# hagabbar/GenNet

Hardware: AMD Instinct MI355X
Metric: waveforms/sec (CNN+GAN step, 2048-sample BBH) (higher is better)
Workload: dtype f32

## Files before the change

### gennet_amd/csrc/conv_epilogue.h

```cpp
#pragma once
#include "common.h"
#ifndef GN_STORE_AUX
#define GN_STORE_AUX 0
#endif

namespace gn {

typedef float f32x16 __attribute__((ext_vector_type(16)));

struct EpiSrd {
  __amdgpu_buffer_rsrc_t y, m, g;
  float ginv;
};
template <int MODE>
__device__ __forceinline__ EpiSrd epi_srd(const ConvArgs& a, int b) {
  EpiSrd s;
  const uintptr_t yp = (uintptr_t)(a.y + (size_t)b * a.Ly * a.Cout);
  const unsigned ylo = __builtin_amdgcn_readfirstlane((unsigned)yp), yhi = __builtin_amdgcn_readfirstlane((unsigned)(yp >> 32));
  const int ybytes = __builtin_amdgcn_readfirstlane(a.Ly * a.Cout * 4);
  s.y = __builtin_amdgcn_make_buffer_rsrc((void*)(((uintptr_t)yhi << 32) | ylo), 0, ybytes, 0x00020000);
  s.m = s.y; s.g = s.y;
  if (MODE == 1 || MODE == 3) {
    const uintptr_t mp = (uintptr_t)((MODE == 1 ? a.mask : a.gmask) + (size_t)b * a.Ly * a.Cout);
    const unsigned mlo = __builtin_amdgcn_readfirstlane((unsigned)mp), mhi = __builtin_amdgcn_readfirstlane((unsigned)(mp >> 32));
// ... 10 lines not shown
template <int ACT, int MODE, int GACT>
__device__ __forceinline__ void epi_store(const ConvArgs& a, const EpiSrd& s, float v, int voff, int soff) {
  if (ACT == GN_ACT_RELU) v = fmaxf(v, 0.f);
  else if (ACT == GN_ACT_LEAKY) v = v > 0.f ? v : a.act_param * v;
  else if (ACT == GN_ACT_TANH) v = gn_tanhf(v);
  else if (ACT != GN_ACT_LINEAR) v = act_apply(v, a.act, a.act_param);
  if (MODE == 1) {
    const unsigned k = __builtin_amdgcn_raw_buffer_load_b8(s.m, voff, soff, 0);
    v = k ? v * a.keep_scale : 0.f;
  }
  if (MODE >= 2) {
    const float gv = __builtin_bit_cast(float, __builtin_amdgcn_raw_buffer_load_b32(s.g, voff * 4, soff * 4, 0));
    if (MODE == 3) {
      const unsigned k = __builtin_amdgcn_raw_buffer_load_b8(s.m, voff, soff, 0);
      const float y0 = gv * s.ginv;
      const float dg = GACT == GN_ACT_LEAKY ? (y0 > 0.f ? 1.f : a.gparam) : act_grad_from_y(y0, a.gact, a.gparam);
      v = k ? v * a.gscale * dg : 0.f;
    } else {
      v *= GACT == GN_ACT_RELU ? (gv > 0.f ? 1.f : 0.f) : act_grad_from_y(gv, a.gact, a.gparam);
    }
  }
  __builtin_amdgcn_raw_buffer_store_b32(__builtin_bit_cast(unsigned, v), s.y, voff * 4, soff * 4, GN_STORE_AUX);
}

template <int ACT, int MODE, int GACT, int WN, int WMT = 2>
__device__ __forceinline__ void pipe_epilogue(const ConvArgs& a, const f32x16 (&acc)[WMT][WN], int b, int m_base, int n_base, int i32, int h, int out_off) {
  const EpiSrd srd = epi_srd<MODE>(a, b);
  const int rowstride = a.t.out_stride * a.Cout;
#pragma unroll
  for (int nt = 0; nt < WN; ++nt) {
    const int n = n_base + nt * 32 + i32;
    const float bias = a.bias ? a.bias[n] : 0.f;
    const int voff = rowstride * (4 * h) + out_off * a.Cout + n;
#pragma unroll
    for (int mt = 0; mt < WMT; ++mt) {
#pragma unroll
      for (int r = 0; r < 16; ++r) {
        const int soff = rowstride * (m_base + mt * 32 + (r & 3) + 8 * (r >> 2));
        epi_store<ACT, MODE, GACT>(a, srd, acc[mt][nt][r] + bias, voff, soff);
      }
    }
  }
}

typedef float f32x4e __attribute__((ext_vector_type(4)));
template <int ACT, int MODE, int GACT, int NT4>
// ... 14 lines not shown
                                                         int mode) {
#define GN_EPI(A_, M_, G_) tile16_epilogue<A_, M_, G_, NT4>(a, acc, b, m_base, n_base, n16, kq, out_off)
  if (mode == 0) {
    switch (a.act) {
      case GN_ACT_LINEAR: GN_EPI(GN_ACT_LINEAR, 0, -1); break;
      case GN_ACT_RELU: GN_EPI(GN_ACT_RELU, 0, -1); break;
      case GN_ACT_LEAKY: GN_EPI(GN_ACT_LEAKY, 0, -1); break;
      case GN_ACT_TANH: GN_EPI(GN_ACT_TANH, 0, -1); break;
      default: GN_EPI(-1, 0, -1); break;
    }
  } else if (mode == 1) {
    if (a.act == GN_ACT_LEAKY) GN_EPI(GN_ACT_LEAKY, 1, -1);
    else GN_EPI(-1, 1, -1);
  } else if (mode == 2) {
    if (a.act == GN_ACT_LINEAR && a.gact == GN_ACT_RELU) GN_EPI(GN_ACT_LINEAR, 2, GN_ACT_RELU);
    else GN_EPI(-1, 2, -1);
  } else {
    if (a.act == GN_ACT_LINEAR && a.gact == GN_ACT_LEAKY) GN_EPI(GN_ACT_LINEAR, 3, GN_ACT_LEAKY);
    else GN_EPI(-1, 3, -1);
  }
#undef GN_EPI
}

template <int WN, int WMT = 2>
__device__ __forceinline__ void pipe_epilogue_dispatch(const ConvArgs& a, const f32x16 (&acc)[WMT][WN], int b, int m_base, int n_base, int i32, int h, int out_off,
                                                       int mode) {
#define GN_EPI(A_, M_, G_) pipe_epilogue<A_, M_, G_, WN, WMT>(a, acc, b, m_base, n_base, i32, h, out_off)
  if (mode == 0) {
    switch (a.act) {
      case GN_ACT_LINEAR: GN_EPI(GN_ACT_LINEAR, 0, -1); break;
      case GN_ACT_RELU: GN_EPI(GN_ACT_RELU, 0, -1); break;
      case GN_ACT_LEAKY: GN_EPI(GN_ACT_LEAKY, 0, -1); break;
      case GN_ACT_TANH: GN_EPI(GN_ACT_TANH, 0, -1); break;
      default: GN_EPI(-1, 0, -1); break;
    }
  } else if (mode == 1) {
    if (a.act == GN_ACT_LEAKY) GN_EPI(GN_ACT_LEAKY, 1, -1);
    else GN_EPI(-1, 1, -1);
  } else if (mode == 2) {
    if (a.act == GN_ACT_LINEAR && a.gact == GN_ACT_RELU) GN_EPI(GN_ACT_LINEAR, 2, GN_ACT_RELU);
    else GN_EPI(-1, 2, -1);
  } else {
    if (a.act == GN_ACT_LINEAR && a.gact == GN_ACT_LEAKY) GN_EPI(GN_ACT_LINEAR, 3, GN_ACT_LEAKY);
    else GN_EPI(-1, 3, -1);
  }
#undef GN_EPI
// ... 32 lines not shown
```

### gennet_amd/csrc/conv_wino.hip

```cpp
#include <stdlib.h>
#include <algorithm>
#include <type_traits>
#include "common.h"
#include "conv_epilogue.h"
#include "wino_common.h"

namespace gn {

struct WinoTaps {
  int wq[5];
};

__global__ void wino_u_kernel(const float* __restrict__ w, float* __restrict__ U, int Cin, int Cout, WinoTaps t) {
  const size_t i = (size_t)blockIdx.x * blockDim.x + threadIdx.x;
  const size_t cc = (size_t)Cin * Cout;
  if (i >= cc) return;
  const int ci = (int)(i / Cout), co = (int)(i % Cout);
  double g[5];
#pragma unroll
  for (int q = 0; q < 5; ++q) g[q] = (double)w[(size_t)t.wq[q] * cc + i];
  float u[6];
  u[0] = (float)g[0];
  u[1] = (float)((g[0] + g[1] + g[2] + g[3] + g[4]) * (1.0 / 3.0));
  u[2] = (float)((g[0] - g[1] + g[2] - g[3] + g[4]) * (1.0 / 3.0));
  u[3] = (float)((16.0 * g[0] + 8.0 * g[1] + 4.0 * g[2] + 2.0 * g[3] + g[4]) * (1.0 / 15.0));
  u[4] = (float)((g[0] - 2.0 * g[1] + 4.0 * g[2] - 8.0 * g[3] + 16.0 * g[4]) * (1.0 / 30.0));
  u[5] = (float)g[4];
  const int chunk = ci >> 3, c = ci & 7, kq = c >> 1, s = c & 1;
  const int tile = co >> 6, nn = co & 63, ct = nn >> 4, n16 = nn & 15, cth = ct >> 1, ctl = ct & 1;
  const size_t base = ((size_t)chunk * (Cout >> 6) + tile) * 3072 + ((cth * 4 + kq) * 16 + n16) * 4 + ctl * 2 + s;
#pragma unroll
  for (int p = 0; p < 6; ++p) U[base + p * 512] = u[p];
}

template <int O, int OP1>
__device__ __forceinline__ void wino_slot_rba(f32x4& c, float a, float b, f32x4& nb0, f32x4& nb1, unsigned addr_b, f32x2 (&d)[6], unsigned addr_a) {
  asm volatile(
      "ds_read_b128 %1, %11 offset:%13\n\t"
      "ds_read_b128 %2, %11 offset:%14\n\t"
      "ds_read_b64 %3, %12\n\t"
      "ds_read_b64 %4, %12 offset:%15\n\t"
      "ds_read_b64 %5, %12 offset:32\n\t"
      "ds_read_b64 %6, %12 offset:%16\n\t"
      "ds_read_b64 %7, %12 offset:64\n\t"
      "ds_read_b64 %8, %12 offset:%17\n\t"
      "s_waitcnt lgkmcnt(8)\n\t"
      "v_mfma_f32_16x16x4_f32 %0, %9, %10, %0"
      : "+v"(c), "=&v"(nb0), "=&v"(nb1), "=&v"(d[0]), "=&v"(d[1]), "=&v"(d[2]), "=&v"(d[3]), "=&v"(d[4]), "=&v"(d[5])
      : "v"(a), "v"(b), "v"(addr_b), "v"(addr_a), "i"(O), "i"(O + 1024), "i"(OP1), "i"(OP1 + 32), "i"(OP1 + 64)
      : "memory");
}
template <int O>
__device__ __forceinline__ void wino_slot_rbw(f32x4& c, float a, float b, f32x4& nb0, f32x4& nb1, unsigned addr_b, f32x2 (&d)[6]) {
  asm volatile(
      "ds_read_b128 %1, %11 offset:%12\n\t"
      "ds_read_b128 %2, %11 offset:%13\n\t"
      "s_waitcnt lgkmcnt(2)\n\t"
      "v_mfma_f32_16x16x4_f32 %0, %9, %10, %0"
      : "+v"(c), "=&v"(nb0), "=&v"(nb1), "+v"(d[0]), "+v"(d[1]), "+v"(d[2]), "+v"(d[3]), "+v"(d[4]), "+v"(d[5])
      : "v"(a), "v"(b), "v"(addr_b), "i"(O), "i"(O + 1024)
      : "memory");
}

template <int RPER, int ABL = 0>
struct WinoChunk {
  template <int NPIECES, int I = 0, class D>
  static __device__ __forceinline__ void run(f32x4 (&acc)[6][4], const f32x2 (&v)[6], f32x2 (&vn)[6], f32x2 (&d)[6], WinoT& t, f32x4 (&B)[2][2], unsigned addr_b,
                                             unsigned addr_b_next, unsigned addr_a, unsigned long long k15, unsigned long long km15, D& dma) {
    if constexpr (I < 48) {
      constexpr int P = I / 8, S = (I / 4) % 2, CT = I % 4;
      f32x4(&bc)[2] = B[P & 1];
      f32x4(&bn)[2] = B[(P + 1) & 1];
      const float bv = bc[CT >> 1][2 * (CT & 1) + S];
      const float av = v[P][S];
      if constexpr ((ABL & 8) != 0) wino_slot(acc[P][CT], av, bv);
      else if constexpr (I == 0) wino_slot_rba<2048, RPER * 32>(acc[0][0], av, bv, bn[0], bn[1], addr_b, d, addr_a);
      else if constexpr (I == 8) wino_slot_rbw<2 * 2048>(acc[1][0], av, bv, bn[0], bn[1], addr_b, d);
      else if constexpr (I == 40) wino_slot_rb<0, 2>(acc[5][0], av, bv, bn[0], bn[1], addr_b_next);
      else if constexpr (I % 8 == 0) wino_slot_rb<(P + 1) * 2048, 2>(acc[P][0], av, bv, bn[0], bn[1], addr_b);
      else wino_slot(acc[P][CT], av, bv);
      if constexpr ((I & 1) && (I >> 1) < NPIECES) dma(std::integral_constant<int, (I >> 1)>{});
      if constexpr (!(ABL & 2)) {
        if constexpr (I == 12) wino_run<0, 5>(d, vn, t, k15, km15);
        if constexpr (I == 24) wino_run<5, 10>(d, vn, t, k15, km15);
        if constexpr (I == 36) wino_run<10, kWinoPieces>(d, vn, t, k15, km15);
      }
      run<NPIECES, I + 1>(acc, v, vn, d, t, B, addr_b, addr_b_next, addr_a, k15, km15, dma);
    }
  }
};

template <int WAVES_M, int ABL = 0>
__global__ __launch_bounds__(64 * WAVES_M, (WAVES_M > 4 ? 1 : 2)) void conv_wino_kernel(ConvArgs a, const float* __restrict__ U, int off0, int m_tiles, int n_tiles,
                                                                                        int patch) {
#if defined(__HIP_DEVICE_COMPILE__)
  constexpr int KC = 8, NP = 6;
  constexpr int TT = WAVES_M * 16;
  constexpr int TN = 64;
  constexpr int NT = 64 * WAVES_M;
  constexpr int RPER = TT + 2;
  constexpr int SLAB = 2 * RPER * KC;
  constexpr int UT = NP * KC * TN;
  constexpr int BUF = SLAB + UT;
  constexpr int STAGE_BYTES = BUF * 4;
  extern __shared__ __attribute__((aligned(16))) float smem[];
  typedef __attribute__((address_space(3))) void* lptr_t;

  const int tid = threadIdx.x, lane = tid & 63, wave = tid >> 6;
  const int n16 = lane & 15, kq = lane >> 4;
  const BlockTile bt = xcd_block_tile(patch, m_tiles, n_tiles);
  const int n_tile = bt.n_tile, m_tile = bt.m_tile, b = bt.b;
  const int t0 = m_tile * TT, n0 = n_tile * TN;

  f32x4 acc[NP][4];
#pragma unroll
  for (int p = 0; p < NP; ++p)
#pragma unroll
    for (int ct = 0; ct < 4; ++ct)
#pragma unroll
      for (int r = 0; r < 4; ++r) acc[p][ct][r] = 0.f;

  const int t_base = 2 * t0 + off0;
  const uintptr_t xbp = (uintptr_t)(a.x + (size_t)b * a.Lin * a.Cin);
  const unsigned xb_lo = __builtin_amdgcn_readfirstlane((unsigned)xbp), xb_hi = __builtin_amdgcn_readfirstlane((unsigned)(xbp >> 32));
  const int xbytes = __builtin_amdgcn_readfirstlane(a.Lin * a.Cin * 4);
  const __amdgpu_buffer_rsrc_t xsrd = __builtin_amdgcn_make_buffer_rsrc((void*)(((uintptr_t)xb_hi << 32) | xb_lo), 0, xbytes, 0x00020000);

// ... 43 lines not shown
  };

  const unsigned lds0 = (unsigned)(uintptr_t)smem;
  const unsigned base_a = lds0 + (wave * 16 + n16) * 32 + kq * 8;
  const unsigned base_b = lds0 + SLAB * 4 + (kq * 16 + n16) * 16;
  const unsigned long long k15 = 0x3fc000003fc00000ull, km15 = 0xbfc00000bfc00000ull;

  const int n_chunks = a.Cin / KC;
  c_next = 0; st_next = 0; dma_all();
  c_next = min(1, n_chunks - 1); st_next = 1; dma_all();
  __syncthreads();

  f32x2 V0[6], V1[6], d[6];
  f32x4 Bq[2][2];
  WinoT tt;
  {
    const char* sb = reinterpret_cast<const char*>(smem);
#pragma unroll
    for (int j = 0; j < 6; ++j) d[j] = *reinterpret_cast<const f32x2*>(sb + (base_a - lds0) + (j & 1) * RPER * 32 + (j >> 1) * 32);
    wino_run<0, kWinoPieces>(d, V0, tt, k15, km15);
    Bq[0][0] = *reinterpret_cast<const f32x4*>(sb + (base_b - lds0));
    Bq[0][1] = *reinterpret_cast<const f32x4*>(sb + (base_b - lds0) + 1024);
  }
  int st = 0;
  in_loop = true;
  for (int ch = 0; ch < n_chunks; ch += 2) {
#pragma unroll
    for (int half = 0; half < 2; ++half) {
      if (half == 1 && ch + 1 >= n_chunks) break;
      const int st1 = st == 2 ? 0 : st + 1, st2 = st1 == 2 ? 0 : st1 + 1;
      c_next = min(ch + half + 2, n_chunks - 1);
      st_next = st2;
      const unsigned addr_a = base_a + st1 * STAGE_BYTES;
      const unsigned addr_b = base_b + st * STAGE_BYTES, addr_b_next = base_b + st1 * STAGE_BYTES;
      if (half == 0) WinoChunk<RPER, ABL>::template run<NPIECES>(acc, V0, V1, d, tt, Bq, addr_b, addr_b_next, addr_a, k15, km15, dma_piece);
      else WinoChunk<RPER, ABL>::template run<NPIECES>(acc, V1, V0, d, tt, Bq, addr_b, addr_b_next, addr_a, k15, km15, dma_piece);
      if constexpr (!(ABL & 4)) __syncthreads();
      st = st1;
    }
  }
  asm volatile("s_nop 15\n\ts_nop 7" : "+v"(acc[5][0]), "+v"(acc[5][1]), "+v"(acc[5][2]), "+v"(acc[5][3]));

  f32x4 out[2][4];
#pragma unroll
  for (int ct = 0; ct < 4; ++ct)
#pragma unroll
    for (int r = 0; r < 4; ++r) {
      out[0][ct][r] = (((acc[0][ct][r] + acc[1][ct][r]) + acc[2][ct][r]) + acc[3][ct][r]) + acc[4][ct][r];
      out[1][ct][r] = __builtin_fmaf(-2.f, acc[4][ct][r], __builtin_fmaf(0.5f, acc[3][ct][r], acc[1][ct][r] - acc[2][ct][r])) + acc[5][ct][r];
    }
  const int m_base = t0 + __builtin_amdgcn_readfirstlane(wave) * 16;
  const int mode = a.gy ? (a.gmask ? 3 : 2) : (a.mask ? 1 : 0);
  ConvArgs a2 = a;
  a2.t.out_stride = 2;
  tile16_epilogue_dispatch<4>(a2, out[0], b, m_base, n0, n16, kq, a.t.out_off, mode);
  tile16_epilogue_dispatch<4>(a2, out[1], b, m_base, n0, n16, kq, a.t.out_off + 1, mode);

  if (a.stat_part) {
    double* red = reinterpret_cast<double*>(smem);
#pragma unroll
    for (int ct = 0; ct < 4; ++ct) {
      const float bias = a.bias ? a.bias[n0 + ct * 16 + n16] : 0.f;
      double s1 = 0.0, s2 = 0.0;
#pragma unroll
      for (int ph = 0; ph < 2; ++ph)
#pragma unroll
        for (int r = 0; r < 4; ++r) {
          const int row = 2 * (m_base + 4 * kq + r) + ph;
          if (row < a.M) {
            const double v = (double)(out[ph][ct][r] + bias);
            s1 += v; s2 += v * v;
          }
        }
      s1 += __shfl_xor(s1, 16, 64); s2 += __shfl_xor(s2, 16, 64);
      s1 += __shfl_xor(s1, 32, 64); s2 += __shfl_xor(s2, 32, 64);
      if (kq == 0) {
        const int slot = (wave * TN + ct * 16 + n16) * 2;
        red[slot] = s1; red[slot + 1] = s2;
      }
    }
    __syncthreads();
    if (tid < TN) {
// ... 6 lines not shown
    }
  }
#endif
}

template <int WAVES_M, int ABL = 0>
static int launch_conv_wino(const ConvArgs& a, const float* U, int off0, hipStream_t s) {
  constexpr int TT = WAVES_M * 16, TN = 64;
  constexpr size_t lds = 3 * sizeof(float) * ((size_t)2 * (TT + 2) * 8 + (size_t)6 * 8 * TN);
  static_assert(lds <= 160 * 1024, "stages too large");
  if (lds > 64 * 1024) {
    static unsigned long long lds_done = 0;
    allow_big_lds((const void*)conv_wino_kernel<WAVES_M, ABL>, &lds_done);
  }
  const int tiles = (a.M + 1) / 2;
  const int m_tiles = (tiles + TT - 1) / TT, n_tiles = a.Cout / TN;
  const size_t blocks = (size_t)m_tiles * n_tiles * a.B;
  if (blocks == 0 || blocks > 0x7fffffffull) {
    set_error("conv_wino: bad grid %zu", blocks);
    return GN_EINVAL;
  }
  const int patch = xcd_patch(n_tiles);
  prof_begin(s);
  hipLaunchKernelGGL((conv_wino_kernel<WAVES_M, ABL>), dim3((unsigned)blocks), dim3(64 * WAVES_M), lds, s, a, U, off0, m_tiles, n_tiles, patch);
  prof_end(s, 0.6 * 2.0 * a.B * (double)a.M * 5 * a.Cin * a.Cout, 5, 4.0 * ((double)a.B * a.Lin * a.Cin + 5.0 * a.Cin * a.Cout + (double)a.B * a.M * a.Cout));
  int rc = check_launch("conv_wino");
  if (rc || !a.stat_part) return rc;
  *a.stat_done = 1;
  return colred_finalize(a.stat_part, a.stat_sums, (size_t)2 * a.Cout, a.B * m_tiles, s);
}

size_t conv_wino_workspace_bytes(int Cin, int Cout) { return (size_t)6 * Cin * Cout * sizeof(float); }

bool conv_wino_supported(const ConvArgs& a) {
  if (a.t.ntaps != 5 || a.t.in_stride != 1 || a.t.out_stride != 1 || a.t.out_off != 0) return false;
  if (a.Cin % 8 || a.Cout % 64 || a.Cin < 8) return false;
  if ((size_t)a.Ly * a.Cout * 4 >= 0x40000000ull || (size_t)a.Lin * a.Cin * 4 >= 0x40000000ull || (size_t)6 * a.Cin * a.Cout * 4 >= 0x40000000ull) return false;
  bool seen[5] = {false, false, false, false, false};
  int minoff = a.t.off[0];
  for (int j = 1; j < 5; ++j) minoff = std::min(minoff, a.t.off[j]);
  for (int j = 0; j < 5; ++j) {
    const int q = a.t.off[j] - minoff;
    if (q < 0 || q > 4 || seen[q]) return false;
    seen[q] = true;
  }
  if (a.stat_part && (a.act != GN_ACT_LINEAR || a.mask || a.gy)) return false;
  return true;
// ... 39 lines not shown
```

### gennet_amd/csrc/conv_wino_s2.hip

```cpp
#include <stdlib.h>
#include <algorithm>
#include <type_traits>
#include "common.h"
#include "conv_epilogue.h"
#include "wino_common.h"

namespace gn {

struct WinoS2Taps {
  int wq[5];
};

__global__ void wino_s2_u_kernel(const float* __restrict__ w, float* __restrict__ U, int Cin, int Cout, WinoS2Taps t) {
  const size_t i = (size_t)blockIdx.x * blockDim.x + threadIdx.x;
  const size_t cc = (size_t)Cin * Cout;
  if (i >= cc) return;
  const int ci = (int)(i / Cout), co = (int)(i % Cout);
  double g[5];
#pragma unroll
  for (int q = 0; q < 5; ++q) g[q] = (double)w[(size_t)t.wq[q] * cc + i];
  float u[7];
  u[0] = (float)g[0];
  u[1] = (float)(0.5 * (g[0] + g[2] + g[4]));
  u[2] = (float)(0.5 * (g[0] - g[2] + g[4]));
  u[3] = (float)g[4];
  u[4] = (float)g[1];
  u[5] = (float)(g[1] + g[3]);
  u[6] = (float)g[3];
  const int chunk = ci >> 3, c = ci & 7, kq = c >> 1, s = c & 1;
  const int tile = co >> 6, nn = co & 63, ct = nn >> 4, n16 = nn & 15, cth = ct >> 1, ctl = ct & 1;
  const size_t base = ((size_t)chunk * (Cout >> 6) + tile) * 3584 + ((cth * 4 + kq) * 16 + n16) * 4 + ctl * 2 + s;
#pragma unroll
  for (int p = 0; p < 7; ++p) U[base + p * 512] = u[p];
}

template <int O, int PB>
__device__ __forceinline__ void s2_slot_rba7(f32x4& c, float a, float b, f32x4& nb0, f32x4& nb1, unsigned addr_b, f32x2 (&d)[7], unsigned addr_a) {
  asm volatile(
      "ds_read_b128 %1, %12 offset:%14\n\t"
      "ds_read_b128 %2, %12 offset:%15\n\t"
      "ds_read_b64 %3, %13\n\t"
      "ds_read_b64 %4, %13 offset:%16\n\t"
      "ds_read_b64 %5, %13 offset:%17\n\t"
      "ds_read_b64 %6, %13 offset:%18\n\t"
      "ds_read_b64 %7, %13 offset:32\n\t"
      "ds_read_b64 %8, %13 offset:%19\n\t"
      "ds_read_b64 %9, %13 offset:%20\n\t"
      "s_waitcnt lgkmcnt(9)\n\t"
      "v_mfma_f32_16x16x4_f32 %0, %10, %11, %0"
      : "+v"(c), "=&v"(nb0), "=&v"(nb1), "=&v"(d[0]), "=&v"(d[1]), "=&v"(d[2]), "=&v"(d[3]), "=&v"(d[4]), "=&v"(d[5]), "=&v"(d[6])
      : "v"(a), "v"(b), "v"(addr_b), "v"(addr_a), "i"(O), "i"(O + 1024), "i"(PB), "i"(2 * PB), "i"(3 * PB), "i"(PB + 32), "i"(2 * PB + 32)
      : "memory");
}
template <int O, int PB>
__device__ __forceinline__ void s2_slot_rba4(f32x4& c, float a, float b, f32x4& nb0, f32x4& nb1, unsigned addr_b, f32x2 (&d)[4], unsigned addr_a) {
  asm volatile(
      "ds_read_b128 %1, %9 offset:%11\n\t"
      "ds_read_b128 %2, %9 offset:%12\n\t"
      "ds_read_b64 %3, %10\n\t"
      "ds_read_b64 %4, %10 offset:%13\n\t"
      "ds_read_b64 %5, %10 offset:32\n\t"
      "ds_read_b64 %6, %10 offset:%14\n\t"
      "s_waitcnt lgkmcnt(6)\n\t"
      "v_mfma_f32_16x16x4_f32 %0, %7, %8, %0"
      : "+v"(c), "=&v"(nb0), "=&v"(nb1), "=&v"(d[0]), "=&v"(d[1]), "=&v"(d[2]), "=&v"(d[3])
      : "v"(a), "v"(b), "v"(addr_b), "v"(addr_a), "i"(O), "i"(O + 1024), "i"(PB), "i"(PB + 32)
      : "memory");
}
template <int O>
__device__ __forceinline__ void s2_slot_rbw7(f32x4& c, float a, float b, f32x4& nb0, f32x4& nb1, unsigned addr_b, f32x2 (&d)[7]) {
  asm volatile(
      "ds_read_b128 %1, %12 offset:%13\n\t"
      "ds_read_b128 %2, %12 offset:%14\n\t"
      "s_waitcnt lgkmcnt(2)\n\t"
      "v_mfma_f32_16x16x4_f32 %0, %10, %11, %0"
      : "+v"(c), "=&v"(nb0), "=&v"(nb1), "+v"(d[0]), "+v"(d[1]), "+v"(d[2]), "+v"(d[3]), "+v"(d[4]), "+v"(d[5]), "+v"(d[6])
      : "v"(a), "v"(b), "v"(addr_b), "i"(O), "i"(O + 1024)
      : "memory");
}
template <int O>
__device__ __forceinline__ void s2_slot_rbw4(f32x4& c, float a, float b, f32x4& nb0, f32x4& nb1, unsigned addr_b, f32x2 (&d)[4]) {
  asm volatile(
      "ds_read_b128 %1, %9 offset:%10\n\t"
      "ds_read_b128 %2, %9 offset:%11\n\t"
      "s_waitcnt lgkmcnt(2)\n\t"
      "v_mfma_f32_16x16x4_f32 %0, %7, %8, %0"
      : "+v"(c), "=&v"(nb0), "=&v"(nb1), "+v"(d[0]), "+v"(d[1]), "+v"(d[2]), "+v"(d[3])
      : "v"(a), "v"(b), "v"(addr_b), "i"(O), "i"(O + 1024)
      : "memory");
}

template <int KIND, int SB, int RPER, int NR, int PAR>
struct S2Chunk {
  template <int NPIECES, int I = 0, class D>
  static __device__ __forceinline__ void run(f32x4 (&acc)[7][4], const f32x2 (&v)[7], f32x2 (&vn)[7], f32x2 (&d)[NR], f32x4 (&B)[2][2], unsigned addr_b,
                                             unsigned addr_b_next, unsigned addr_a, D& dma) {
    if constexpr (I < 56) {
      constexpr int P = I / 8, S = (I / 4) % 2, CT = I % 4;
      f32x4(&bc)[2] = B[(P + PAR) & 1];
      f32x4(&bn)[2] = B[(P + PAR + 1) & 1];
      const float bv = bc[CT >> 1][2 * (CT & 1) + S];
      const float av = v[P][S];
      if constexpr (I == 0) {
        if constexpr (NR == 7) s2_slot_rba7<2048, RPER * 32>(acc[0][0], av, bv, bn[0], bn[1], addr_b, d, addr_a);
        else s2_slot_rba4<2048, RPER * 32>(acc[0][0], av, bv, bn[0], bn[1], addr_b, d, addr_a);
      } else if constexpr (I == 8) {
        if constexpr (NR == 7) s2_slot_rbw7<2 * 2048>(acc[1][0], av, bv, bn[0], bn[1], addr_b, d);
        else s2_slot_rbw4<2 * 2048>(acc[1][0], av, bv, bn[0], bn[1], addr_b, d);
      } else if constexpr (I == 48) wino_slot_rb<0, 2>(acc[6][0], av, bv, bn[0], bn[1], addr_b_next);
      else if constexpr (I % 8 == 0) wino_slot_rb<(P + 1) * 2048, 2>(acc[P][0], av, bv, bn[0], bn[1], addr_b);
      else wino_slot(acc[P][CT], av, bv);
      if constexpr ((I & 1) && (I >> 1) < NPIECES) dma(std::integral_constant<int, (I >> 1)>{});
      if constexpr (I == 20) s2_run<KIND, SB, NR, 0, 4>(d, vn);
      if constexpr (I == 36) s2_run<KIND, SB, NR, 4, 7>(d, vn);
      run<NPIECES, I + 1>(acc, v, vn, d, B, addr_b, addr_b_next, addr_a, dma);
    }
  }
};

template <int KIND, int SB>
__global__ __launch_bounds__(256, 2) void conv_wino_s2_kernel(ConvArgs a, const float* __restrict__ U, int off0, int m_tiles, int n_tiles, int patch, int offA,
                                                              int offB) {
#if defined(__HIP_DEVICE_COMPILE__)
  constexpr int KC = 8, NP = 7, WAVES_M = 4;
  constexpr int TT = WAVES_M * 16, TN = 64, NT = 64 * WAVES_M;
  constexpr int NR = KIND == 1 ? 7 : 4;
  constexpr int TS = KIND == 1 ? 4 : 2;
  constexpr int RPER = TT + 1;
  constexpr int SLAB = TS * RPER * KC;
  constexpr int UT = NP * KC * TN;
  constexpr int BUF = SLAB + UT;
  constexpr int STAGE_BYTES = BUF * 4;
  extern __shared__ __attribute__((aligned(16))) float smem[];
  typedef __attribute__((address_space(3))) void* lptr_t;

  const int tid = threadIdx.x, lane = tid & 63, wave = tid >> 6;
  const int n16 = lane & 15, kq = lane >> 4;
  const BlockTile bt = xcd_block_tile(patch, m_tiles, n_tiles);
  const int n_tile = bt.n_tile, m_tile = bt.m_tile, b = bt.b;
  const int t0 = m_tile * TT, n0 = n_tile * TN;

  f32x4 acc[NP][4];
#pragma unroll
  for (int p = 0; p < NP; ++p)
#pragma unroll
    for (int ct = 0; ct < 4; ++ct)
#pragma unroll
      for (int r = 0; r < 4; ++r) acc[p][ct][r] = 0.f;

  const int t_base = TS * t0 + off0;
  const uintptr_t xbp = (uintptr_t)(a.x + (size_t)b * a.Lin * a.Cin);
  const unsigned xb_lo = __builtin_amdgcn_readfirstlane((unsigned)xbp), xb_hi = __builtin_amdgcn_readfirstlane((unsigned)(xbp >> 32));
  const int xbytes = __builtin_amdgcn_readfirstlane(a.Lin * a.Cin * 4);
  const __amdgpu_buffer_rsrc_t xsrd = __builtin_amdgcn_make_buffer_rsrc((void*)(((uintptr_t)xb_hi << 32) | xb_lo), 0, xbytes, 0x00020000);

// ... 41 lines not shown
    if constexpr (NPIECES > 6) dma_piece(std::integral_constant<int, 6>{});
    if constexpr (NPIECES > 7) dma_piece(std::integral_constant<int, 7>{});
  };

  const unsigned lds0 = (unsigned)(uintptr_t)smem;
  const unsigned base_a = lds0 + (wave * 16 + n16) * 32 + kq * 8;
  const unsigned base_b = lds0 + SLAB * 4 + (kq * 16 + n16) * 16;

  const int n_chunks = a.Cin / KC;
  c_next = 0; st_next = 0; dma_all();
  c_next = min(1, n_chunks - 1); st_next = 1; dma_all();
  __syncthreads();

  f32x2 V0[7], V1[7], d[NR];
  f32x4 Bq[2][2];
  {
    const char* sb = reinterpret_cast<const char*>(smem);
#pragma unroll
    for (int j = 0; j < NR; ++j) d[j] = *reinterpret_cast<const f32x2*>(sb + (base_a - lds0) + (j % TS) * RPER * 32 + (j / TS) * 32);
    s2_run<KIND, SB, NR, 0, 7>(d, V0);
    Bq[0][0] = *reinterpret_cast<const f32x4*>(sb + (base_b - lds0));
    Bq[0][1] = *reinterpret_cast<const f32x4*>(sb + (base_b - lds0) + 1024);
  }
  int st = 0;
  for (int ch = 0; ch < n_chunks; ch += 2) {
#pragma unroll
    for (int half = 0; half < 2; ++half) {
      if (half == 1 && ch + 1 >= n_chunks) break;
      const int st1 = st == 2 ? 0 : st + 1, st2 = st1 == 2 ? 0 : st1 + 1;
      c_next = min(ch + half + 2, n_chunks - 1);
      st_next = st2;
      const unsigned addr_a = base_a + st1 * STAGE_BYTES;
      const unsigned addr_b = base_b + st * STAGE_BYTES, addr_b_next = base_b + st1 * STAGE_BYTES;
      if (half == 0) S2Chunk<KIND, SB, RPER, NR, 0>::template run<NPIECES>(acc, V0, V1, d, Bq, addr_b, addr_b_next, addr_a, dma_piece);
      else S2Chunk<KIND, SB, RPER, NR, 1>::template run<NPIECES>(acc, V1, V0, d, Bq, addr_b, addr_b_next, addr_a, dma_piece);
      __syncthreads();
      st = st1;
    }
  }
  asm volatile("s_nop 15\n\ts_nop 7" : "+v"(acc[6][0]), "+v"(acc[6][1]), "+v"(acc[6][2]), "+v"(acc[6][3]));

  const int m_base = t0 + __builtin_amdgcn_readfirstlane(wave) * 16;
  const int mode = a.gy ? (a.gmask ? 3 : 2) : (a.mask ? 1 : 0);
  ConvArgs a2 = a;
  if constexpr (KIND == 1) {
    f32x4 out[2][4];
#pragma unroll
    for (int ct = 0; ct < 4; ++ct)
#pragma unroll
      for (int r = 0; r < 4; ++r) {
        out[0][ct][r] = ((acc[0][ct][r] + acc[1][ct][r]) + acc[2][ct][r]) + (acc[4][ct][r] + acc[5][ct][r]);
        out[1][ct][r] = ((acc[1][ct][r] - acc[2][ct][r]) - acc[3][ct][r]) + (acc[5][ct][r] + acc[6][ct][r]);
      }
    a2.t.out_stride = 2;
    tile16_epilogue_dispatch<4>(a2, out[0], b, m_base, n0, n16, kq, a.t.out_off, mode);
    tile16_epilogue_dispatch<4>(a2, out[1], b, m_base, n0, n16, kq, a.t.out_off + 1, mode);
    if (a.stat_part) {
      double* red = reinterpret_cast<double*>(smem);
#pragma unroll
      for (int ct = 0; ct < 4; ++ct) {
        const float bias = a.bias ? a.bias[n0 + ct * 16 + n16] : 0.f;
        double s1 = 0.0, s2 = 0.0;
#pragma unroll
        for (int ph = 0; ph < 2; ++ph)
#pragma unroll
          for (int r = 0; r < 4; ++r) {
            const int row = 2 * (m_base + 4 * kq + r) + ph;
            if (row < a.M) {
              const double v = (double)(out[ph][ct][r] + bias);
              s1 += v; s2 += v * v;
            }
          }
        s1 += __shfl_xor(s1, 16, 64); s2 += __shfl_xor(s2, 16, 64);
        s1 += __shfl_xor(s1, 32, 64); s2 += __shfl_xor(s2, 32, 64);
        if (kq == 0) {
          const int slot = (wave * TN + ct * 16 + n16) * 2;
          red[slot] = s1; red[slot + 1] = s2;
        }
      }
      __syncthreads();
      if (tid < TN) {
        double t1 = 0.0, t2 = 0.0;
#pragma unroll
        for (int w = 0; w < WAVES_M; ++w) { t1 += red[(w * TN + tid) * 2]; t2 += red[(w * TN + tid) * 2 + 1]; }
        double* dst = a.stat_part + (size_t)(b * m_tiles + m_tile) * 2 * a.Cout;
        dst[n0 + tid] = t1;
        dst[a.Cout + n0 + tid] = t2;
      }
    }
  } else {
    f32x4 out[4][4];
#pragma unroll
    for (int ct = 0; ct < 4; ++ct)
#pragma unroll
      for (int r = 0; r < 4; ++r) {
        out[0][ct][r] = (acc[0][ct][r] + acc[1][ct][r]) + acc[2][ct][r];
        out[1][ct][r] = (acc[1][ct][r] - acc[2][ct][r]) - acc[3][ct][r];
        out[2][ct][r] = acc[4][ct][r] + acc[5][ct][r];
        out[3][ct][r] = acc[5][ct][r] + acc[6][ct][r];
      }
    a2.t.out_stride = 4;
    tile16_epilogue_dispatch<4>(a2, out[0], b, m_base, n0, n16, kq, offA, mode);
    tile16_epilogue_dispatch<4>(a2, out[1], b, m_base, n0, n16, kq, offA + 2, mode);
    tile16_epilogue_dispatch<4>(a2, out[2], b, m_base, n0, n16, kq, offB, mode);
    tile16_epilogue_dispatch<4>(a2, out[3], b, m_base, n0, n16, kq, offB + 2, mode);
  }
#endif
}

template <int KIND, int SB>
static int launch_s2(const ConvArgs& a, const float* U, int off0, int offA, int offB, hipStream_t s) {
  constexpr int TT = 64, TN = 64, TS = KIND == 1 ? 4 : 2;
  constexpr size_t lds = 3 * sizeof(float) * ((size_t)TS * (TT + 1) * 8 + (size_t)7 * 8 * TN);
  static_assert(lds <= 160 * 1024, "stages too large");
  if (lds > 64 * 1024) {
    static unsigned long long lds_done = 0;
    allow_big_lds((const void*)conv_wino_s2_kernel<KIND, SB>, &lds_done);
  }
  const int tiles = (a.M + 1) / 2;
  const int m_tiles = (tiles + TT - 1) / TT, n_tiles = a.Cout / TN;
  const size_t blocks = (size_t)m_tiles * n_tiles * a.B;
  if (blocks == 0 || blocks > 0x7fffffffull) {
    set_error("conv_wino_s2: bad grid %zu", blocks);
    return GN_EINVAL;
  }
  const int patch = xcd_patch(n_tiles);
  prof_begin(s);
  hipLaunchKernelGGL((conv_wino_s2_kernel<KIND, SB>), dim3((unsigned)blocks), dim3(256), lds, s, a, U, off0, m_tiles, n_tiles, patch, offA, offB);
  prof_end(s, 0.7 * 2.0 * a.B * (double)a.M * 5 * a.Cin * a.Cout, 7, 4.0 * ((double)a.B * a.Lin * a.Cin + 5.0 * a.Cin * a.Cout + (double)a.B * a.M * a.Cout));
  int rc = check_launch("conv_wino_s2");
  if (rc || !a.stat_part) return rc;
  *a.stat_done = 1;
  return colred_finalize(a.stat_part, a.stat_sums, (size_t)2 * a.Cout, a.B * m_tiles, s);
}

size_t conv_wino_s2_workspace_bytes(int Cin, int Cout) { return (size_t)7 * Cin * Cout * sizeof(float); }

int conv_wino_s2_kind(const ConvArgs& a) {
  if (a.t.ntaps != 5 || a.Cin % 8 || a.Cout % 64 || a.Cin < 32) return 0;
  if ((size_t)a.Ly * a.Cout * 4 >= 0x40000000ull || (size_t)a.Lin * a.Cin * 4 >= 0x40000000ull || (size_t)7 * a.Cin * a.Cout * 4 >= 0x40000000ull) return 0;
  if (a.t.in_stride == 2 && a.t.out_stride == 1 && a.t.out_off == 0) {
    for (int j = 0; j < 5; ++j)
      if (a.t.off[j] != a.t.off[0] + j) return 0;
    if (a.stat_part && (a.act != GN_ACT_LINEAR || a.mask || a.gy)) return 0;
    return 1;
  }
  if (a.t.in_stride == 1 && a.t.out_stride == 2 && !a.stat_part && !a.mask && !a.bias) {
    if (a.t.off[0] != a.t.off[2] + 1 || a.t.off[2] != a.t.off[4] + 1 || a.t.off[1] != a.t.off[3] + 1) return 0;
    const int sb = a.t.off[3] - a.t.off[4];
    if (sb != 0 && sb != 1) return 0;
    return 2;
// ... 37 lines not shown
```

Measured before the change: 1964.

## Add LDS-staged wide-store epilogue and unroll Winograd chunk loop by three stages

Adds a wide epilogue that stages each wave's output tile through LDS, then reads it back and writes 128-bit vector stores (with 32-bit mask and 128-bit gradient loads) in place of scalar 32-bit stores. It also unrolls the main Winograd chunk loop six-at-a-time so that stage offsets become compile-time immediates in the ds_read instructions, removing per-chunk address arithmetic. The wide path is selected at launch only when the pointers are aligned. In exchange it spends extra LDS traffic and waits in the epilogue, moves the stats reduction area in shared memory, and grows code size.

```diff
diff --git a/gennet_amd/csrc/conv_epilogue.h b/gennet_amd/csrc/conv_epilogue.h
--- a/gennet_amd/csrc/conv_epilogue.h
+++ b/gennet_amd/csrc/conv_epilogue.h
@@ -56,6 +56,22 @@
   }
   __builtin_amdgcn_raw_buffer_store_b32(__builtin_bit_cast(unsigned, v), s.y, voff * 4, soff * 4, GN_STORE_AUX);
 }
+template <int ACT, int MODE, int GACT>
+__device__ __forceinline__ float epi_value(const ConvArgs& a, const EpiSrd& s, float v, unsigned k, float gv) {
+  if (ACT == GN_ACT_RELU) v = fmaxf(v, 0.f);
+  else if (ACT == GN_ACT_LEAKY) v = v > 0.f ? v : a.act_param * v;
+  else if (ACT == GN_ACT_TANH) v = gn_tanhf(v);
+  else if (ACT != GN_ACT_LINEAR) v = act_apply(v, a.act, a.act_param);
+  if (MODE == 1) v = k ? v * a.keep_scale : 0.f;
+  if (MODE == 3) {
+    const float y0 = gv * s.ginv;
+    const float dg = GACT == GN_ACT_LEAKY ? (y0 > 0.f ? 1.f : a.gparam) : act_grad_from_y(y0, a.gact, a.gparam);
+    v = k ? v * a.gscale * dg : 0.f;
+  } else if (MODE == 2) {
+    v *= GACT == GN_ACT_RELU ? (gv > 0.f ? 1.f : 0.f) : act_grad_from_y(gv, a.gact, a.gparam);
+  }
+  return v;
+}
 
 template <int ACT, int MODE, int GACT, int WN, int WMT = 2>
 __device__ __forceinline__ void pipe_epilogue(const ConvArgs& a, const f32x16 (&acc)[WMT][WN], int b, int m_base, int n_base, int i32, int h, int out_off) {
@@ -116,6 +132,81 @@
 #undef GN_EPI
 }
 
+typedef unsigned u32x4e __attribute__((ext_vector_type(4)));
+constexpr int kWideEpiFloats = 2 * 16 * 64;
+template <int ACT, int MODE, int GACT>
+__device__ __forceinline__ void tile16_wide_epilogue(const ConvArgs& a, const f32x4e (&o0)[4], const f32x4e (&o1)[4], float* wreg, int b, int m_base, int n_base,
+                                                     int lane, int off0, int off1) {
+  const EpiSrd srd = epi_srd<MODE>(a, b);
+  const int rowstride = a.t.out_stride * a.Cout;
+  const int n16 = lane & 15, kq = lane >> 4;
+  float* wr = wreg + (4 * kq) * 64 + n16;
+  float bias[4] = {0.f, 0.f, 0.f, 0.f};
+  if (a.bias) {
+#pragma unroll
+    for (int ct = 0; ct < 4; ++ct) bias[ct] = a.bias[n_base + ct * 16 + n16];
+  }
+#pragma unroll
+  for (int ct = 0; ct < 4; ++ct) {
+#pragma unroll
+    for (int r = 0; r < 4; ++r) {
+      wr[r * 64 + ct * 16] = o0[ct][r] + bias[ct];
+      wr[1024 + r * 64 + ct * 16] = o1[ct][r] + bias[ct];
+    }
+  }
+  asm volatile("s_waitcnt lgkmcnt(0)" ::: "memory");
+  const int c4 = 4 * n16;
+  const float* rd = wreg + kq * 64 + c4;
+  const int voff = rowstride * kq + n_base + c4;
+#pragma unroll
+  for (int ph = 0; ph < 2; ++ph) {
+#pragma unroll
+    for (int g = 0; g < 4; ++g) {
+      f32x4e v = *reinterpret_cast<const f32x4e*>(rd + ph * 1024 + g * 256);
+      const int soff = rowstride * (m_base + 4 * g) + (ph ? off1 : off0) * a.Cout;
+      unsigned k4 = 0;
+      u32x4e g4 = {0u, 0u, 0u, 0u};
+      if (MODE == 1 || MODE == 3) k4 = __builtin_amdgcn_raw_buffer_load_b32(srd.m, voff, soff, 0);
+      if (MODE >= 2) g4 = __builtin_amdgcn_raw_buffer_load_b128(srd.g, voff * 4, soff * 4, 0);
+      u32x4e o;
+#pragma unroll
+      for (int e = 0; e < 4; ++e) {
+        const float ve = v[e];
+        const unsigned ge = g4[e];
+        o[e] = __builtin_bit_cast(unsigned, epi_value<ACT, MODE, GACT>(a, srd, ve, (k4 >> (8 * e)) & 0xffu, __builtin_bit_cast(float, ge)));
+      }
+      __builtin_amdgcn_raw_buffer_store_b128(o, srd.y, voff * 4, soff * 4, GN_STORE_AUX);
+    }
+  }
+}
+__device__ __forceinline__ void tile16_wide_epilogue_dispatch(const ConvArgs& a, const f32x4e (&o0)[4], const f32x4e (&o1)[4], float* wreg, int b, int m_base,
+                                                              int n_base, int lane, int off0, int off1, int mode) {
+#define GN_EPI(A_, M_, G_) tile16_wide_epilogue<A_, M_, G_>(a, o0, o1, wreg, b, m_base, n_base, lane, off0, off1)
+  if (mode == 0) {
+    switch (a.act) {
+      case GN_ACT_LINEAR: GN_EPI(GN_ACT_LINEAR, 0, -1); break;
+      case GN_ACT_RELU: GN_EPI(GN_ACT_RELU, 0, -1); break;
+      case GN_ACT_LEAKY: GN_EPI(GN_ACT_LEAKY, 0, -1); break;
+      case GN_ACT_TANH: GN_EPI(GN_ACT_TANH, 0, -1); break;
+      default: GN_EPI(-1, 0, -1); break;
+    }
+  } else if (mode == 1) {
+    if (a.act == GN_ACT_LEAKY) GN_EPI(GN_ACT_LEAKY, 1, -1);
+    else GN_EPI(-1, 1, -1);
+  } else if (mode == 2) {
+    if (a.act == GN_ACT_LINEAR && a.gact == GN_ACT_RELU) GN_EPI(GN_ACT_LINEAR, 2, GN_ACT_RELU);
+    else GN_EPI(-1, 2, -1);
+  } else {
+    if (a.act == GN_ACT_LINEAR && a.gact == GN_ACT_LEAKY) GN_EPI(GN_ACT_LINEAR, 3, GN_ACT_LEAKY);
+    else GN_EPI(-1, 3, -1);
+  }
+#undef GN_EPI
+}
+static inline bool wide_epilogue_aligned(const ConvArgs& a) {
+  const uintptr_t mk = (uintptr_t)(a.gy ? a.gmask : a.mask);
+  return (uintptr_t)a.y % 16 == 0 && (uintptr_t)a.gy % 16 == 0 && mk % 4 == 0;
+}
+
 template <int WN, int WMT = 2>
 __device__ __forceinline__ void pipe_epilogue_dispatch(const ConvArgs& a, const f32x16 (&acc)[WMT][WN], int b, int m_base, int n_base, int i32, int h, int out_off,
                                                        int mode) {
diff --git a/gennet_amd/csrc/conv_wino.hip b/gennet_amd/csrc/conv_wino.hip
--- a/gennet_amd/csrc/conv_wino.hip
+++ b/gennet_amd/csrc/conv_wino.hip
@@ -33,21 +33,22 @@
   for (int p = 0; p < 6; ++p) U[base + p * 512] = u[p];
 }
 
-template <int O, int OP1>
+template <int O, int OP1, int OA = 0>
 __device__ __forceinline__ void wino_slot_rba(f32x4& c, float a, float b, f32x4& nb0, f32x4& nb1, unsigned addr_b, f32x2 (&d)[6], unsigned addr_a) {
   asm volatile(
       "ds_read_b128 %1, %11 offset:%13\n\t"
       "ds_read_b128 %2, %11 offset:%14\n\t"
-      "ds_read_b64 %3, %12\n\t"
+      "ds_read_b64 %3, %12 offset:%18\n\t"
       "ds_read_b64 %4, %12 offset:%15\n\t"
-      "ds_read_b64 %5, %12 offset:32\n\t"
+      "ds_read_b64 %5, %12 offset:%19\n\t"
       "ds_read_b64 %6, %12 offset:%16\n\t"
-      "ds_read_b64 %7, %12 offset:64\n\t"
+      "ds_read_b64 %7, %12 offset:%20\n\t"
       "ds_read_b64 %8, %12 offset:%17\n\t"
       "s_waitcnt lgkmcnt(8)\n\t"
       "v_mfma_f32_16x16x4_f32 %0, %9, %10, %0"
       : "+v"(c), "=&v"(nb0), "=&v"(nb1), "=&v"(d[0]), "=&v"(d[1]), "=&v"(d[2]), "=&v"(d[3]), "=&v"(d[4]), "=&v"(d[5])
-      : "v"(a), "v"(b), "v"(addr_b), "v"(addr_a), "i"(O), "i"(O + 1024), "i"(OP1), "i"(OP1 + 32), "i"(OP1 + 64)
+      : "v"(a), "v"(b), "v"(addr_b), "v"(addr_a), "i"(O), "i"(O + 1024), "i"(OA + OP1), "i"(OA + OP1 + 32), "i"(OA + OP1 + 64), "i"(OA), "i"(OA + 32),
+        "i"(OA + 64)
       : "memory");
 }
 template <int O>
@@ -62,7 +63,7 @@
       : "memory");
 }
 
-template <int RPER, int ABL = 0>
+template <int RPER, int ABL = 0, int OB = 0, int OBN = 0, int OA = 0>
 struct WinoChunk {
   template <int NPIECES, int I = 0, class D>
   static __device__ __forceinline__ void run(f32x4 (&acc)[6][4], const f32x2 (&v)[6], f32x2 (&vn)[6], f32x2 (&d)[6], WinoT& t, f32x4 (&B)[2][2], unsigned addr_b,
@@ -74,10 +75,10 @@
       const float bv = bc[CT >> 1][2 * (CT & 1) + S];
       const float av = v[P][S];
       if constexpr ((ABL & 8) != 0) wino_slot(acc[P][CT], av, bv);
-      else if constexpr (I == 0) wino_slot_rba<2048, RPER * 32>(acc[0][0], av, bv, bn[0], bn[1], addr_b, d, addr_a);
-      else if constexpr (I == 8) wino_slot_rbw<2 * 2048>(acc[1][0], av, bv, bn[0], bn[1], addr_b, d);
-      else if constexpr (I == 40) wino_slot_rb<0, 2>(acc[5][0], av, bv, bn[0], bn[1], addr_b_next);
-      else if constexpr (I % 8 == 0) wino_slot_rb<(P + 1) * 2048, 2>(acc[P][0], av, bv, bn[0], bn[1], addr_b);
+      else if constexpr (I == 0) wino_slot_rba<OB + 2048, RPER * 32, OA>(acc[0][0], av, bv, bn[0], bn[1], addr_b, d, addr_a);
+      else if constexpr (I == 8) wino_slot_rbw<OB + 2 * 2048>(acc[1][0], av, bv, bn[0], bn[1], addr_b, d);
+      else if constexpr (I == 40) wino_slot_rb<OBN, 2>(acc[5][0], av, bv, bn[0], bn[1], addr_b_next);
+      else if constexpr (I % 8 == 0) wino_slot_rb<OB + (P + 1) * 2048, 2>(acc[P][0], av, bv, bn[0], bn[1], addr_b);
       else wino_slot(acc[P][CT], av, bv);
       if constexpr ((I & 1) && (I >> 1) < NPIECES) dma(std::integral_constant<int, (I >> 1)>{});
       if constexpr (!(ABL & 2)) {
@@ -92,7 +93,7 @@
 
 template <int WAVES_M, int ABL = 0>
 __global__ __launch_bounds__(64 * WAVES_M, (WAVES_M > 4 ? 1 : 2)) void conv_wino_kernel(ConvArgs a, const float* __restrict__ U, int off0, int m_tiles, int n_tiles,
-                                                                                        int patch) {
+                                                                                        int patch, int wide) {
 #if defined(__HIP_DEVICE_COMPILE__)
   constexpr int KC = 8, NP = 6;
   constexpr int TT = WAVES_M * 16;
@@ -103,6 +104,8 @@
   constexpr int UT = NP * KC * TN;
   constexpr int BUF = SLAB + UT;
   constexpr int STAGE_BYTES = BUF * 4;
+  constexpr int RED = WAVES_M * kWideEpiFloats;
+  static_assert(RED * 4 + WAVES_M * TN * 16 <= 3 * STAGE_BYTES, "epilogue regions");
   extern __shared__ __attribute__((aligned(16))) float smem[];
   typedef __attribute__((address_space(3))) void* lptr_t;
 
@@ -192,9 +195,27 @@
     Bq[0][0] = *reinterpret_cast<const f32x4*>(sb + (base_b - lds0));
     Bq[0][1] = *reinterpret_cast<const f32x4*>(sb + (base_b - lds0) + 1024);
   }
-  int st = 0;
+  int st = 0, ch = 0;
   in_loop = true;
-  for (int ch = 0; ch < n_chunks; ch += 2) {
+  static_assert(2 * STAGE_BYTES + 6 * 2048 + RPER * 32 + 64 < 65536, "stage offsets as ds_read immediates");
+  auto chunk_of_six = [&](auto jc) {
+    constexpr int J = decltype(jc)::value, S0 = J % 3, S1 = (J + 1) % 3, S2 = (J + 2) % 3;
+    c_next = min(ch + J + 2, n_chunks - 1);
+    st_next = S2;
+    using Chunk = WinoChunk<RPER, ABL, S0 * STAGE_BYTES, S1 * STAGE_BYTES, S1 * STAGE_BYTES>;
+    if constexpr (J % 2 == 0) Chunk::template run<NPIECES>(acc, V0, V1, d, tt, Bq, base_b, base_b, base_a, k15, km15, dma_piece);
+    else Chunk::template run<NPIECES>(acc, V1, V0, d, tt, Bq, base_b, base_b, base_a, k15, km15, dma_piece);
+    if constexpr (!(ABL & 4)) __syncthreads();
+  };
+  for (; ch + 6 <= n_chunks; ch += 6) {
+    chunk_of_six(std::integral_constant<int, 0>{});
+    chunk_of_six(std::integral_constant<int, 1>{});
+    chunk_of_six(std::integral_constant<int, 2>{});
+    chunk_of_six(std::integral_constant<int, 3>{});
+    chunk_of_six(std::integral_constant<int, 4>{});
+    chunk_of_six(std::integral_constant<int, 5>{});
+  }
+  for (; ch < n_chunks; ch += 2) {
 #pragma unroll
     for (int half = 0; half < 2; ++half) {
       if (half == 1 && ch + 1 >= n_chunks) break;
@@ -209,7 +230,7 @@
       st = st1;
     }
   }
-  asm volatile("s_nop 15\n\ts_nop 7" : "+v"(acc[5][0]), "+v"(acc[5][1]), "+v"(acc[5][2]), "+v"(acc[5][3]));
+  asm volatile("s_waitcnt lgkmcnt(0)\n\ts_nop 15\n\ts_nop 7" : "+v"(acc[5][0]), "+v"(acc[5][1]), "+v"(acc[5][2]), "+v"(acc[5][3]));
 
   f32x4 out[2][4];
 #pragma unroll
@@ -223,11 +244,16 @@
   const int mode = a.gy ? (a.gmask ? 3 : 2) : (a.mask ? 1 : 0);
   ConvArgs a2 = a;
   a2.t.out_stride = 2;
-  tile16_epilogue_dispatch<4>(a2, out[0], b, m_base, n0, n16, kq, a.t.out_off, mode);
-  tile16_epilogue_dispatch<4>(a2, out[1], b, m_base, n0, n16, kq, a.t.out_off + 1, mode);
+  if (wide) {
+    tile16_wide_epilogue_dispatch(a2, out[0], out[1], smem + __builtin_amdgcn_readfirstlane(wave) * kWideEpiFloats, b, m_base, n0, lane, a.t.out_off,
+                                  a.t.out_off + 1, mode);
+  } else {
+    tile16_epilogue_dispatch<4>(a2, out[0], b, m_base, n0, n16, kq, a.t.out_off, mode);
+    tile16_epilogue_dispatch<4>(a2, out[1], b, m_base, n0, n16, kq, a.t.out_off + 1, mode);
+  }
 
   if (a.stat_part) {
-    double* red = reinterpret_cast<double*>(smem);
+    double* red = reinterpret_cast<double*>(smem + RED);
 #pragma unroll
     for (int ct = 0; ct < 4; ++ct) {
       const float bias = a.bias ? a.bias[n0 + ct * 16 + n16] : 0.f;
@@ -280,7 +306,8 @@
   }
   const int patch = xcd_patch(n_tiles);
   prof_begin(s);
-  hipLaunchKernelGGL((conv_wino_kernel<WAVES_M, ABL>), dim3((unsigned)blocks), dim3(64 * WAVES_M), lds, s, a, U, off0, m_tiles, n_tiles, patch);
+  hipLaunchKernelGGL((conv_wino_kernel<WAVES_M, ABL>), dim3((unsigned)blocks), dim3(64 * WAVES_M), lds, s, a, U, off0, m_tiles, n_tiles, patch,
+                     wide_epilogue_aligned(a) ? 1 : 0);
   prof_end(s, 0.6 * 2.0 * a.B * (double)a.M * 5 * a.Cin * a.Cout, 5, 4.0 * ((double)a.B * a.Lin * a.Cin + 5.0 * a.Cin * a.Cout + (double)a.B * a.M * a.Cout));
   int rc = check_launch("conv_wino");
   if (rc || !a.stat_part) return rc;
diff --git a/gennet_amd/csrc/conv_wino_s2.hip b/gennet_amd/csrc/conv_wino_s2.hip
--- a/gennet_amd/csrc/conv_wino_s2.hip
+++ b/gennet_amd/csrc/conv_wino_s2.hip
@@ -34,37 +34,38 @@
   for (int p = 0; p < 7; ++p) U[base + p * 512] = u[p];
 }
 
-template <int O, int PB>
+template <int O, int PB, int OA = 0>
 __device__ __forceinline__ void s2_slot_rba7(f32x4& c, float a, float b, f32x4& nb0, f32x4& nb1, unsigned addr_b, f32x2 (&d)[7], unsigned addr_a) {
   asm volatile(
       "ds_read_b128 %1, %12 offset:%14\n\t"
       "ds_read_b128 %2, %12 offset:%15\n\t"
-      "ds_read_b64 %3, %13\n\t"
+      "ds_read_b64 %3, %13 offset:%21\n\t"
       "ds_read_b64 %4, %13 offset:%16\n\t"
       "ds_read_b64 %5, %13 offset:%17\n\t"
       "ds_read_b64 %6, %13 offset:%18\n\t"
-      "ds_read_b64 %7, %13 offset:32\n\t"
+      "ds_read_b64 %7, %13 offset:%22\n\t"
       "ds_read_b64 %8, %13 offset:%19\n\t"
       "ds_read_b64 %9, %13 offset:%20\n\t"
       "s_waitcnt lgkmcnt(9)\n\t"
       "v_mfma_f32_16x16x4_f32 %0, %10, %11, %0"
       : "+v"(c), "=&v"(nb0), "=&v"(nb1), "=&v"(d[0]), "=&v"(d[1]), "=&v"(d[2]), "=&v"(d[3]), "=&v"(d[4]), "=&v"(d[5]), "=&v"(d[6])
-      : "v"(a), "v"(b), "v"(addr_b), "v"(addr_a), "i"(O), "i"(O + 1024), "i"(PB), "i"(2 * PB), "i"(3 * PB), "i"(PB + 32), "i"(2 * PB + 32)
+      : "v"(a), "v"(b), "v"(addr_b), "v"(addr_a), "i"(O), "i"(O + 1024), "i"(OA + PB), "i"(OA + 2 * PB), "i"(OA + 3 * PB), "i"(OA + PB + 32),
+        "i"(OA + 2 * PB + 32), "i"(OA), "i"(OA + 32)
       : "memory");
 }
-template <int O, int PB>
+template <int O, int PB, int OA = 0>
 __device__ __forceinline__ void s2_slot_rba4(f32x4& c, float a, float b, f32x4& nb0, f32x4& nb1, unsigned addr_b, f32x2 (&d)[4], unsigned addr_a) {
   asm volatile(
       "ds_read_b128 %1, %9 offset:%11\n\t"
       "ds_read_b128 %2, %9 offset:%12\n\t"
-      "ds_read_b64 %3, %10\n\t"
+      "ds_read_b64 %3, %10 offset:%15\n\t"
       "ds_read_b64 %4, %10 offset:%13\n\t"
-      "ds_read_b64 %5, %10 offset:32\n\t"
+      "ds_read_b64 %5, %10 offset:%16\n\t"
       "ds_read_b64 %6, %10 offset:%14\n\t"
       "s_waitcnt lgkmcnt(6)\n\t"
       "v_mfma_f32_16x16x4_f32 %0, %7, %8, %0"
       : "+v"(c), "=&v"(nb0), "=&v"(nb1), "=&v"(d[0]), "=&v"(d[1]), "=&v"(d[2]), "=&v"(d[3])
-      : "v"(a), "v"(b), "v"(addr_b), "v"(addr_a), "i"(O), "i"(O + 1024), "i"(PB), "i"(PB + 32)
+      : "v"(a), "v"(b), "v"(addr_b), "v"(addr_a), "i"(O), "i"(O + 1024), "i"(OA + PB), "i"(OA + PB + 32), "i"(OA), "i"(OA + 32)
       : "memory");
 }
 template <int O>
@@ -90,7 +91,7 @@
       : "memory");
 }
 
-template <int KIND, int SB, int RPER, int NR, int PAR>
+template <int KIND, int SB, int RPER, int NR, int PAR, int OB = 0, int OBN = 0, int OA = 0>
 struct S2Chunk {
   template <int NPIECES, int I = 0, class D>
   static __device__ __forceinline__ void run(f32x4 (&acc)[7][4], const f32x2 (&v)[7], f32x2 (&vn)[7], f32x2 (&d)[NR], f32x4 (&B)[2][2], unsigned addr_b,
@@ -102,13 +103,13 @@
       const float bv = bc[CT >> 1][2 * (CT & 1) + S];
       const float av = v[P][S];
       if constexpr (I == 0) {
-        if constexpr (NR == 7) s2_slot_rba7<2048, RPER * 32>(acc[0][0], av, bv, bn[0], bn[1], addr_b, d, addr_a);
-        else s2_slot_rba4<2048, RPER * 32>(acc[0][0], av, bv, bn[0], bn[1], addr_b, d, addr_a);
+        if constexpr (NR == 7) s2_slot_rba7<OB + 2048, RPER * 32, OA>(acc[0][0], av, bv, bn[0], bn[1], addr_b, d, addr_a);
+        else s2_slot_rba4<OB + 2048, RPER * 32, OA>(acc[0][0], av, bv, bn[0], bn[1], addr_b, d, addr_a);
       } else if constexpr (I == 8) {
-        if constexpr (NR == 7) s2_slot_rbw7<2 * 2048>(acc[1][0], av, bv, bn[0], bn[1], addr_b, d);
-        else s2_slot_rbw4<2 * 2048>(acc[1][0], av, bv, bn[0], bn[1], addr_b, d);
-      } else if constexpr (I == 48) wino_slot_rb<0, 2>(acc[6][0], av, bv, bn[0], bn[1], addr_b_next);
-      else if constexpr (I % 8 == 0) wino_slot_rb<(P + 1) * 2048, 2>(acc[P][0], av, bv, bn[0], bn[1], addr_b);
+        if constexpr (NR == 7) s2_slot_rbw7<OB + 2 * 2048>(acc[1][0], av, bv, bn[0], bn[1], addr_b, d);
+        else s2_slot_rbw4<OB + 2 * 2048>(acc[1][0], av, bv, bn[0], bn[1], addr_b, d);
+      } else if constexpr (I == 48) wino_slot_rb<OBN, 2>(acc[6][0], av, bv, bn[0], bn[1], addr_b_next);
+      else if constexpr (I % 8 == 0) wino_slot_rb<OB + (P + 1) * 2048, 2>(acc[P][0], av, bv, bn[0], bn[1], addr_b);
       else wino_slot(acc[P][CT], av, bv);
       if constexpr ((I & 1) && (I >> 1) < NPIECES) dma(std::integral_constant<int, (I >> 1)>{});
       if constexpr (I == 20) s2_run<KIND, SB, NR, 0, 4>(d, vn);
@@ -120,7 +121,7 @@
 
 template <int KIND, int SB>
 __global__ __launch_bounds__(256, 2) void conv_wino_s2_kernel(ConvArgs a, const float* __restrict__ U, int off0, int m_tiles, int n_tiles, int patch, int offA,
-                                                              int offB) {
+                                                              int offB, int wide) {
 #if defined(__HIP_DEVICE_COMPILE__)
   constexpr int KC = 8, NP = 7, WAVES_M = 4;
   constexpr int TT = WAVES_M * 16, TN = 64, NT = 64 * WAVES_M;
@@ -131,6 +132,8 @@
   constexpr int UT = NP * KC * TN;
   constexpr int BUF = SLAB + UT;
   constexpr int STAGE_BYTES = BUF * 4;
+  constexpr int RED = WAVES_M * kWideEpiFloats;
+  static_assert(RED * 4 + WAVES_M * TN * 16 <= 3 * STAGE_BYTES, "epilogue regions");
   extern __shared__ __attribute__((aligned(16))) float smem[];
   typedef __attribute__((address_space(3))) void* lptr_t;
 
@@ -218,8 +221,26 @@
     Bq[0][0] = *reinterpret_cast<const f32x4*>(sb + (base_b - lds0));
     Bq[0][1] = *reinterpret_cast<const f32x4*>(sb + (base_b - lds0) + 1024);
   }
-  int st = 0;
-  for (int ch = 0; ch < n_chunks; ch += 2) {
+  int st = 0, ch = 0;
+  static_assert(2 * STAGE_BYTES + 6 * 2048 + 1024 < 65536 && 2 * STAGE_BYTES + 3 * RPER * 32 + 32 < 65536, "stage offsets as ds_read immediates");
+  auto chunk_of_six = [&](auto jc) {
+    constexpr int J = decltype(jc)::value, S0 = J % 3, S1 = (J + 1) % 3, S2 = (J + 2) % 3;
+    c_next = min(ch + J + 2, n_chunks - 1);
+    st_next = S2;
+    using Chunk = S2Chunk<KIND, SB, RPER, NR, J % 2, S0 * STAGE_BYTES, S1 * STAGE_BYTES, S1 * STAGE_BYTES>;
+    if constexpr (J % 2 == 0) Chunk::template run<NPIECES>(acc, V0, V1, d, Bq, base_b, base_b, base_a, dma_piece);
+    else Chunk::template run<NPIECES>(acc, V1, V0, d, Bq, base_b, base_b, base_a, dma_piece);
+    __syncthreads();
+  };
+  for (; ch + 6 <= n_chunks; ch += 6) {
+    chunk_of_six(std::integral_constant<int, 0>{});
+    chunk_of_six(std::integral_constant<int, 1>{});
+    chunk_of_six(std::integral_constant<int, 2>{});
+    chunk_of_six(std::integral_constant<int, 3>{});
+    chunk_of_six(std::integral_constant<int, 4>{});
+    chunk_of_six(std::integral_constant<int, 5>{});
+  }
+  for (; ch < n_chunks; ch += 2) {
 #pragma unroll
     for (int half = 0; half < 2; ++half) {
       if (half == 1 && ch + 1 >= n_chunks) break;
@@ -234,11 +255,12 @@
       st = st1;
     }
   }
-  asm volatile("s_nop 15\n\ts_nop 7" : "+v"(acc[6][0]), "+v"(acc[6][1]), "+v"(acc[6][2]), "+v"(acc[6][3]));
+  asm volatile("s_waitcnt lgkmcnt(0)\n\ts_nop 15\n\ts_nop 7" : "+v"(acc[6][0]), "+v"(acc[6][1]), "+v"(acc[6][2]), "+v"(acc[6][3]));
 
   const int m_base = t0 + __builtin_amdgcn_readfirstlane(wave) * 16;
   const int mode = a.gy ? (a.gmask ? 3 : 2) : (a.mask ? 1 : 0);
   ConvArgs a2 = a;
+  float* wreg = smem + __builtin_amdgcn_readfirstlane(wave) * kWideEpiFloats;
   if constexpr (KIND == 1) {
     f32x4 out[2][4];
 #pragma unroll
@@ -249,10 +271,14 @@
         out[1][ct][r] = ((acc[1][ct][r] - acc[2][ct][r]) - acc[3][ct][r]) + (acc[5][ct][r] + acc[6][ct][r]);
       }
     a2.t.out_stride = 2;
-    tile16_epilogue_dispatch<4>(a2, out[0], b, m_base, n0, n16, kq, a.t.out_off, mode);
-    tile16_epilogue_dispatch<4>(a2, out[1], b, m_base, n0, n16, kq, a.t.out_off + 1, mode);
+    if (wide) {
+      tile16_wide_epilogue_dispatch(a2, out[0], out[1], wreg, b, m_base, n0, lane, a.t.out_off, a.t.out_off + 1, mode);
+    } else {
+      tile16_epilogue_dispatch<4>(a2, out[0], b, m_base, n0, n16, kq, a.t.out_off, mode);
+      tile16_epilogue_dispatch<4>(a2, out[1], b, m_base, n0, n16, kq, a.t.out_off + 1, mode);
+    }
     if (a.stat_part) {
-      double* red = reinterpret_cast<double*>(smem);
+      double* red = reinterpret_cast<double*>(smem + RED);
 #pragma unroll
       for (int ct = 0; ct < 4; ++ct) {
         const float bias = a.bias ? a.bias[n0 + ct * 16 + n16] : 0.f;
@@ -296,10 +322,15 @@
         out[3][ct][r] = acc[5][ct][r] + acc[6][ct][r];
       }
     a2.t.out_stride = 4;
-    tile16_epilogue_dispatch<4>(a2, out[0], b, m_base, n0, n16, kq, offA, mode);
-    tile16_epilogue_dispatch<4>(a2, out[1], b, m_base, n0, n16, kq, offA + 2, mode);
-    tile16_epilogue_dispatch<4>(a2, out[2], b, m_base, n0, n16, kq, offB, mode);
-    tile16_epilogue_dispatch<4>(a2, out[3], b, m_base, n0, n16, kq, offB + 2, mode);
+    if (wide) {
+      tile16_wide_epilogue_dispatch(a2, out[0], out[1], wreg, b, m_base, n0, lane, offA, offA + 2, mode);
+      tile16_wide_epilogue_dispatch(a2, out[2], out[3], wreg, b, m_base, n0, lane, offB, offB + 2, mode);
+    } else {
+      tile16_epilogue_dispatch<4>(a2, out[0], b, m_base, n0, n16, kq, offA, mode);
+      tile16_epilogue_dispatch<4>(a2, out[1], b, m_base, n0, n16, kq, offA + 2, mode);
+      tile16_epilogue_dispatch<4>(a2, out[2], b, m_base, n0, n16, kq, offB, mode);
+      tile16_epilogue_dispatch<4>(a2, out[3], b, m_base, n0, n16, kq, offB + 2, mode);
+    }
   }
 #endif
 }
@@ -322,7 +353,8 @@
   }
   const int patch = xcd_patch(n_tiles);
   prof_begin(s);
-  hipLaunchKernelGGL((conv_wino_s2_kernel<KIND, SB>), dim3((unsigned)blocks), dim3(256), lds, s, a, U, off0, m_tiles, n_tiles, patch, offA, offB);
+  hipLaunchKernelGGL((conv_wino_s2_kernel<KIND, SB>), dim3((unsigned)blocks), dim3(256), lds, s, a, U, off0, m_tiles, n_tiles, patch, offA, offB,
+                     wide_epilogue_aligned(a) ? 1 : 0);
   prof_end(s, 0.7 * 2.0 * a.B * (double)a.M * 5 * a.Cin * a.Cout, 7, 4.0 * ((double)a.B * a.Lin * a.Cin + 5.0 * a.Cin * a.Cout + (double)a.B * a.M * a.Cout));
   int rc = check_launch("conv_wino_s2");
   if (rc || !a.stat_part) return rc;
```

Measured after the change: 1996, median of 6. 1.02x the previous value.
